# althonos/pyskani

Hardware: AMD Instinct MI355X
Metric: genome-pairs/sec (sketch+ANI) (higher is better)
Workload: dtype u64; 1 GPU; all-vs-all 10000 x 10000 synthetic ~5 Mb genomes on one GPU (100 families x 100; single-contig genomes, substitutions only), c=125 marker_c=1000 k=15; device-resident ASCII; hits=999867, genomes=10000, parallelism=references sharded over 1 GPU(s)

## Files before the change

pyskani_amd/csrc/chain.hip:

```cpp
#include "chain_stages.h"
#include "query_parts.h"
#include <hipcub/hipcub.hpp>
#include <cmath>
#include <algorithm>
#include <unordered_map>


SketchDesc make_desc(const psk_sketch* s, bool unindexed_ok) {
    SketchDesc d{};
    const bool ix = s->idx != nullptr;
    d.key = ix ? s->idx->km32 + s->idx_off : nullptr; d.pms = ix ? s->idx->pms + s->idx_off : nullptr;
    d.perm = ix ? s->idx->perm + s->idx_off : nullptr; d.bucket = ix ? s->idx->bucket + s->idx_boff : nullptr;
    d.bshift = ix ? s->idx_bshift : 0; d.n = (ix || (unindexed_ok && s->store)) ? (uint32_t)s->n_seeds : 0;
    d.pos = s->store ? s->store->seed_pos + s->seed_off : nullptr; d.meta = s->store ? s->store->seed_meta + s->seed_off : nullptr;
    d.kmer = s->store ? s->store->seed_kmer + s->seed_off : nullptr;
    d.seed_pos_base = s->store ? s->store->seed_pos : nullptr;
    d.contig_start = s->store ? s->store->contig_seed_start + s->contig_off : nullptr;
    d.total_len = s->total_len; d.n_contigs = (uint32_t)s->contig_len.size();
    uint64_t rows = 0;
    if (d.n) for (uint32_t len : s->contig_len) rows += (uint64_t)len / (FRAGMENT_LENGTH + 1) + 1;
    d.rows = (uint32_t)std::min<uint64_t>(rows, 0xFFFFFFFFu);
    s->len_quantiles(d.lenq);
    d.tab = (ix && s->ptab) ? (const ProbeLine*)s->ptab->base + s->ptab_off : nullptr; d.tab_lines = (ix && s->ptab) ? s->ptab_lines : 0;
    return d;
// ... 98 lines not shown
__global__ __launch_bounds__(256) void work_rows_kernel(const ChunkOut* __restrict__ cout, const uint32_t* __restrict__ n_chunks, const uint32_t* __restrict__ cbase,
                                                        const uint32_t* __restrict__ row_pair, uint32_t n_rows, unsigned long long* __restrict__ out) {
    __shared__ unsigned long long s_c[4], s_l[4];
    unsigned long long c = 0, live = 0;
    for (uint32_t r = blockIdx.x * blockDim.x + threadIdx.x; r < n_rows; r += gridDim.x * blockDim.x) {
        const uint32_t p = row_pair[r];
        if (r - cbase[p] < n_chunks[p]) { c += cout[r].n_cand; live++; }
    }
#pragma unroll
    for (int o = 32; o > 0; o >>= 1) { c += __shfl_xor(c, o); live += __shfl_xor(live, o); }
    if ((threadIdx.x & 63) == 0) { s_c[threadIdx.x >> 6] = c; s_l[threadIdx.x >> 6] = live; }
    __syncthreads();
    if (threadIdx.x == 0) {
        c = s_c[0] + s_c[1] + s_c[2] + s_c[3]; live = s_l[0] + s_l[1] + s_l[2] + s_l[3];
        if (live) { atomicAdd(&out[0], c); atomicAdd(&out[1], live); }
    }
}

psk_status chain_layout(Lane* ctx, size_t n_pairs, size_t n_items, size_t n_rows, size_t n_bq, ChainBufs* L) {
    const size_t gi = (n_items + 255) / 256, gi_sum = std::max(gi, (n_pairs + 3) / 4);
    size_t o_pairs = 0, o_sbase = al256(o_pairs + sizeof(PairDesc) * n_pairs), o_cbase = al256(o_sbase + 4 * (n_pairs + 1)),
           o_pstart = al256(o_cbase + 4 * (n_pairs + 1)), o_lb = al256(o_pstart + 4 * (n_pairs + 1)),
           o_aoff = al256(o_lb + 8 * (n_items + 1)), o_nch = al256(o_aoff + 4 * (n_items + 1)),
           o_chunks = al256(o_nch + 4 * n_pairs), o_rq0 = al256(o_chunks + sizeof(uint2) * n_rows), o_cout = al256(o_rq0 + sizeof(uint2) * n_rows),
           o_misc = al256(o_cout + sizeof(ChunkOut) * n_rows), o_hits = o_misc + 256, o_sel = al256(o_hits + sizeof(psk_hit) * n_pairs),
           o_ovf = al256(o_sel + sizeof(psk_hit) * n_pairs), o_bsum = al256(o_ovf + 4 * n_rows),
           o_qr = al256(o_bsum + 8 * (gi_sum + 1)), o_bq = al256(o_qr + 8 * n_pairs), o_bp = al256(o_bq + sizeof(BatchQ) * (n_bq + 1)),
           o_rp = al256(o_bp + 4 * (gi + 1)), o_live = al256(o_rp + 4 * (n_rows + 1)), o_big = al256(o_live + 4 * (n_pairs + 1)),
           o_huge = al256(o_big + 4 * (n_pairs + 1)), o_end = o_huge + 4 * (n_pairs + 1);
    PSK_TRY(ctx->q_b.reserve(o_end));
    char* B = (char*)ctx->q_b.p;
    L->pairs = (PairDesc*)(B + o_pairs); L->sbase = (uint32_t*)(B + o_sbase); L->cbase = (uint32_t*)(B + o_cbase); L->pstart = (uint32_t*)(B + o_pstart);
    L->lbcnt = (uint2*)(B + o_lb); L->aoff = (uint32_t*)(B + o_aoff); L->nch = (uint32_t*)(B + o_nch); L->chunks = (uint2*)(B + o_chunks); L->row_q0 = (uint2*)(B + o_rq0);
    L->cout = (ChunkOut*)(B + o_cout); L->hits = (psk_hit*)(B + o_hits); L->hits_sel = (psk_hit*)(B + o_sel); L->misc = (uint32_t*)(B + o_misc);
    L->ovf = (uint32_t*)(B + o_ovf); L->bsum = (unsigned long long*)(B + o_bsum); L->pair_qr = (uint2*)(B + o_qr); L->bq = (BatchQ*)(B + o_bq);
    L->blk_pair = (uint32_t*)(B + o_bp); L->row_pair = (uint32_t*)(B + o_rp); L->live = (uint32_t*)(B + o_live); L->big_list = (uint32_t*)(B + o_big); L->huge_list = (uint32_t*)(B + o_huge);
    L->gi = (uint32_t)gi; L->gi_sum = (uint32_t)gi_sum;
    L->total = (unsigned long long*)(L->misc + 16);
    return PSK_OK;
}

psk_status chain_run(Lane* ctx, const ChainBufs& L, uint32_t n_pairs, size_t n_items, size_t n_rows, const psk_params& prm,
                     const psk_query_opts* o, const SketchDesc* d_qd, const SketchDesc* d_rd, uint64_t cap, bool wide, const Switches& sw, bool probe_ok) {
    hipStream_t st = ctx->stream;
    const int force_serial = sw.chain_serial.get() != nullptr;
    const uint32_t gi = L.gi;
    hipLaunchKernelGGL(pair_table_kernel, dim3((uint32_t)(((size_t)gi + n_rows + 255) / 256)), dim3(256), 0, st, L.sbase, L.cbase, n_pairs, gi, (uint32_t)n_items, (uint32_t)n_rows, L.blk_pair, L.row_pair,
                       L.misc, L.lbcnt + n_items);
    ctx->t_begin(K_ANCHOR);
    if (wide) hipLaunchKernelGGL(anchor_count_kernel, dim3(gi), dim3(256), 0, st, L.pairs, L.sbase, n_pairs, (uint32_t)n_items, L.lbcnt, L.bsum, L.blk_pair);
    const uint32_t gi4 = (gi + JT - 1) / JT;
    uint32_t n_sum = gi;
    const int jp_force = sw.join_pairs.force();
    const bool gsi_join = !wide && (L.g_key || L.b_key) && L.d_pass && L.n_bq;
    const bool join_pairs = !wide && (gsi_join || (jp_force >= 0 ? jp_force == 1 : (n_pairs >= 16384 && n_items / n_pairs < 2048)));
    const bool gsl = gsi_join && L.gsi_slice;
    const bool gsi_one = gsi_join && !gsl && L.gsi_onepass && cap >= n_items + n_items / 8 + 8 * ((size_t)n_pairs + 1);
    bool probe_local = false;
    GsiJoinArgs GA{};
    GslArgs GL{};
    const uint32_t gsi_nw = (L.g_key && !L.gsi_slice) ? std::max(4u, (L.n_refs + 63u) / 64u) : 4u;
    const size_t gsi_lds_row = 8 * (size_t)gsi_nw + 4 * (size_t)((gsi_nw + 1u) & ~1u), gsi_lds_count = gsi_lds_row + 4 * (size_t)L.p_cap, gsi_lds_emit = gsi_lds_row + 4 * (size_t)L.p_cap * 9;
    if (gsi_join) {
        GA.bq = L.bq; GA.pass = L.d_pass; GA.n_refs = L.n_refs; GA.qd = d_qd; GA.g_key = L.g_key; GA.g_val = L.g_val; GA.g_bucket = L.g_bucket; GA.g_shift = L.g_shift;
        GA.b_key = L.b_key; GA.b_val = L.b_val; GA.b_bucket = L.b_bucket; GA.b_shift = L.b_shift; GA.b_nb1 = L.b_nb1; GA.b_blocks = L.b_blocks; GA.b_max = L.b_max;
        GA.pair_cnt = L.big_list; GA.pstart = L.pstart; GA.cap = (uint32_t)cap; GA.err = L.misc; GA.p_cap = L.p_cap; GA.nw_lds = gsi_nw;
        const uint32_t t_blocks = gsl ? L.g_blocks : L.b_blocks;
        const unsigned long long* t_base = gsl ? L.g_base : L.b_base;
        const uint32_t bcap = std::max(1u, std::min<uint32_t>(t_blocks, std::min<uint32_t>(GSI_PMAX, std::max(1u, L.p_cap))));
        uint32_t* d_btab = nullptr; uint32_t* d_bcnt = nullptr;
        if (t_blocks) {
            const size_t o_bc = al256(4 * (size_t)L.n_bq * bcap * GSL_BT_WORDS);
            PSK_TRY(ctx->q_k.reserve(o_bc + 4 * (size_t)L.n_bq + 256));
            d_btab = (uint32_t*)ctx->q_k.p; d_bcnt = (uint32_t*)((char*)ctx->q_k.p + o_bc);
            PSK_TRY(gsl_blocks_launch(L.bq, L.n_bq, L.d_pass, L.n_refs, t_blocks, t_base, d_btab, d_bcnt, bcap, st));
        }
        GA.blk_tab = d_btab; GA.blk_cnt = d_bcnt; GA.blk_cap = bcap;
        if (gsl) {
            GL.bq = L.bq; GL.n_entries = L.n_bq; GL.tab = L.gsl_tab; GL.n_tab = L.gsl_n_tab; GL.ebase = L.gsl_ebase; GL.pass = L.d_pass; GL.n_refs = L.n_refs; GL.qd = d_qd;
            GL.g_key = L.g_key; GL.g_val = L.g_val; GL.g_bucket = L.g_bucket; GL.g_shift = L.g_shift; GL.g_nb1 = L.g_nb1; GL.g_blocks = L.g_blocks; GL.g_base = L.g_base; GL.blk_tab = d_btab; GL.blk_cnt = d_bcnt; GL.blk_cap = bcap; GL.cnt = L.gsl_cnt; GL.rec = L.gsl_rec; GL.bm = L.gsl_bm; GL.un = L.gsl_un; GL.n_slices = L.gsl_n_slices;
            GL.pair_cnt = L.big_list; GL.pstart = L.pstart; GL.cap = (uint32_t)cap; GL.err = L.misc; GL.p_cap = L.p_cap; GL.chunks = L.chunks; GL.n_chunks = L.nch; GL.row_q0 = L.row_q0;
            PSK_HIP(hipMemsetAsync(L.big_list, 0, 4 * ((size_t)n_pairs + 1), st));
            PSK_TRY(gsl_count_launch(GL, st));
        }
        else if (!gsi_one) hipLaunchKernelGGL(gsi_join_kernel<false>, dim3(L.n_bq), dim3(64), gsi_lds_count, st, GA);
        probe_local = true;
    }
    else if (join_pairs) {
        size_t ts = 0;
        uint32_t* keys_in = L.big_list;
        uint32_t* vals_in = L.live;
        uint32_t* keys_out = (uint32_t*)L.hits_sel;
        uint32_t* order = keys_out + n_pairs;
        hipLaunchKernelGGL(pair_ref_keys_kernel, dim3((n_pairs + 255) / 256), dim3(256), 0, st, L.pair_qr, n_pairs, keys_in, vals_in);
        PSK_HIP(hipcub::DeviceRadixSort::SortPairs(nullptr, ts, keys_in, keys_out, vals_in, order, (int)n_pairs, 0, 32, st));
        PSK_TRY(ctx->q_g.reserve(ts + 256));
        PSK_HIP(hipcub::DeviceRadixSort::SortPairs(ctx->q_g.p, ts, keys_in, keys_out, vals_in, order, (int)n_pairs, 0, 32, st));
        const uint32_t nb = (n_pairs + 3) / 4;
        probe_local = probe_ok;
        if (probe_ok) hipLaunchKernelGGL(anchor_join_probe_kernel, dim3(nb), dim3(256), 0, st, L.pairs, L.sbase, order, n_pairs, L.lbcnt, L.bsum, L.misc + 5, L.aoff, L.big_list);
        else hipLaunchKernelGGL(anchor_join_pairs_kernel, dim3(nb), dim3(256), 0, st, L.pairs, L.sbase, order, n_pairs, L.lbcnt, L.bsum, L.misc + 5);
        n_sum = nb;
    }
    const int ep_force = sw.emit_pairs.force();
    const bool emit_pairs = !wide && !join_pairs && n_items >= 2 * ((size_t)n_pairs + 1) &&
// ... 12 lines not shown
    size_t tmp3 = 0;
    PSK_HIP(hipcub::DeviceSelect::If(nullptr, tmp3, L.hits, L.hits_sel, L.misc + 12, (int)n_pairs, HitPasses(), st));
    PSK_TRY(ctx->q_c.reserve(std::max(tmp, std::max(tmp2, tmp3))));
    unsigned long long* poff = (unsigned long long*)L.aoff;
    hipcub::TransformInputIterator<unsigned long long, Widen, const uint32_t*> pc_it(pair_cnt, Widen());
    if (gsi_one) {
        hipLaunchKernelGGL(gsi_room_kernel, dim3((n_pairs + 1 + 255) / 256), dim3(256), 0, st, (const uint32_t*)L.sbase, n_pairs, L.pstart);
        PSK_HIP(hipMemsetAsync(L.total, 0, 8, st));
    }
    else if (emit_pairs) {
        size_t tmp4 = 0;
        PSK_HIP(hipcub::DeviceScan::ExclusiveSum(nullptr, tmp4, pc_it, poff, (int)(n_pairs + 1), st));
        PSK_TRY(ctx->q_c.reserve(std::max(tmp4, std::max(tmp, std::max(tmp2, tmp3)))));
        PSK_HIP(hipcub::DeviceScan::ExclusiveSum(ctx->q_c.p, tmp4, pc_it, poff, (int)(n_pairs + 1), st));
        hipLaunchKernelGGL(pair_start64_kernel, dim3((n_pairs + 1 + 255) / 256), dim3(256), 0, st, poff, n_pairs, L.pstart, (uint32_t)cap, (const uint32_t*)(L.misc + 5));
    }
    else if (probe_local) {
        hipcub::TransformInputIterator<unsigned long long, Widen, const uint32_t*> pl_it(L.big_list, Widen());
        size_t tmp5 = 0;
        PSK_HIP(hipcub::DeviceScan::ExclusiveSum(nullptr, tmp5, pl_it, (unsigned long long*)nullptr, (int)(n_pairs + 1), st));
        const size_t o_poff = al256(tmp5 + 256);
        PSK_TRY(ctx->q_g.reserve(o_poff + 8 * ((size_t)n_pairs + 2) + 256));
        unsigned long long* pl_off64 = (unsigned long long*)((char*)ctx->q_g.p + o_poff);
        PSK_HIP(hipMemsetAsync(L.big_list + n_pairs, 0, 4, st));
        PSK_HIP(hipcub::DeviceScan::ExclusiveSum(ctx->q_g.p, tmp5, pl_it, pl_off64, (int)(n_pairs + 1), st));
        hipLaunchKernelGGL(pair_start64_kernel, dim3((n_pairs + 1 + 255) / 256), dim3(256), 0, st, (const unsigned long long*)pl_off64, n_pairs, L.pstart, (uint32_t)cap, (const uint32_t*)(L.misc + 5));
        if (gsi_join) hipLaunchKernelGGL(gsi_total_kernel, dim3(1), dim3(1), 0, st, (const unsigned long long*)pl_off64, n_pairs, L.total);
    }
    else if (wide) PSK_HIP(hipcub::DeviceScan::ExclusiveSum(ctx->q_c.p, tmp, cnt_it, L.aoff, (int)(n_items + 1), st));
    else PSK_HIP(hipcub::DeviceScan::ExclusiveSum(ctx->q_c.p, tmp, pcnt_it, L.aoff, (int)(n_items + 1), st));
    const bool small_sum = !gsi_join && n_sum <= 16384;
    if (!small_sum && !gsi_join) PSK_HIP(hipcub::DeviceReduce::Sum(ctx->q_c.p, tmp2, L.bsum, L.total, (int)n_sum, st));
    if ((!emit_pairs && !probe_local) || small_sum)
        hipLaunchKernelGGL(pair_start_kernel, dim3((emit_pairs || probe_local) ? 1u : (n_pairs + 1 + 255) / 256), dim3(256), 0, st, (emit_pairs || probe_local) ? (const uint32_t*)nullptr : L.aoff, L.sbase, n_pairs, L.pstart, (uint32_t)cap,
                           L.bsum, small_sum ? n_sum : 0u, L.total, (const uint32_t*)(L.misc + 5));
    hipLaunchKernelGGL(pair_guard_kernel, dim3((n_pairs + 1 + 255) / 256), dim3(256), 0, st, (const uint32_t*)(L.misc + 5), (const unsigned long long*)L.total, (unsigned long long)cap, L.pstart, n_pairs);
    const size_t na = ((size_t)cap + 64 + 63) & ~(size_t)63;
    PSK_TRY(ctx->q_d.reserve(4 * na * CHAIN_ANCHOR_WORDS));
    PSK_TRY(ctx->q_e.reserve(na * (8 + 4 * 7 + 1) + 512 + 4 * 2 * BIG_GMAX * (BIG_GROUPS + 64) + 4 * BIG_GROUPS));
    uint32_t* D = (uint32_t*)ctx->q_d.p;
    uint32_t* E4 = (uint32_t*)ctx->q_e.p;
    uint4* anc = (uint4*)D;
    uint32_t* a_nxt = D + 4 * na;
    ChainArgs A{};
    A.anc = anc;
    A.row_q0 = gsl ? L.row_q0 : nullptr;
    A.sc_ptr = D + 5 * na;
    A.sc_f = (int32_t*)E4; A.sc_root = E4 + na; A.sc_depth = E4 + 2 * na; A.sc_best = E4 + 3 * na;
    uint32_t* CAND = D + 6 * na;
    A.c_score.p = (int32_t*)CAND; A.c_q0.p = CAND + 1; A.c_q1.p = CAND + 2; A.c_r0.p = CAND + 3; A.c_r1.p = CAND + 4; A.c_n.p = CAND + 5; A.c_rc.p = CAND + 6; A.c_state.p = CAND + 7;
    A.chunks = L.chunks; A.n_chunks = L.nch; A.cbase = L.cbase; A.n_pairs = n_pairs; A.n_rows = (uint32_t)n_rows;
    A.row_pair = L.row_pair;
    A.pairs = L.pairs;
    A.out = L.cout; A.two_c = 2u * (uint32_t)prm.c; A.force_serial = force_serial; A.stats = L.misc + 1;
    A.band = std::max(1, std::min(MAX_CHAIN_BAND, BP_CHAIN_BAND / (int)prm.c));
    A.cap = (uint32_t)cap;
    const bool use_hops = gsi_join ? false : sw.chunk_hops.get() ? !sw.chunk_hops.off() : ((n_pairs < 1024 && n_items / n_pairs > 4096) || n_items / n_pairs > (1u << 20));
    const bool emit_heads = emit_pairs && !use_hops && !sw.emit_heads.off();
    const int hi_force = sw.hops_items.force();
    const bool hops_items = use_hops && !gsl && !emit_pairs && !join_pairs && n_items <= 0x7FFFFFFFull && (hi_force >= 0 ? hi_force == 1 : n_items / n_pairs > (1u << 20));
    ctx->t_begin(K_ANCHOR_EMIT);
    if (hops_items) {
        const size_t o_scr = al256(4 * (size_t)n_pairs * HOP_SLICES + 256);
        PSK_TRY(ctx->q_g.reserve(o_scr + sizeof(uint2) * n_rows + 256));
        uint32_t* slice_cnt = (uint32_t*)ctx->q_g.p;
        uint2* scratch_rows = (uint2*)((char*)ctx->q_g.p + o_scr);
        hipStream_t sd = nullptr;
        PSK_TRY(ctx->side_lane(&sd));
// ... 325 lines not shown
```

pyskani_amd/csrc/chain_stages.h:

```cpp
#pragma once
#include "common.h"
#include "chain_dev.h"
#include "slice_join.h"

struct PairDesc {
    const uint32_t* r_key; const uint64_t* r_pms;
    const uint32_t* q_key; const uint32_t* q_perm;
    const uint32_t* q_pos; const uint32_t* q_meta;
    const uint32_t* q_kmer;
    uint32_t q_nc, pad_;
    const uint32_t* q_seed_pos_base;
    const uint32_t* q_contig_start;
    uint64_t q_total_len, r_total_len;
    uint32_t r_n, q_n;
    const uint32_t* r_bucket; uint32_t r_bshift;
    uint32_t r_tab_lines; const ProbeLine* r_tab;
};


__device__ __forceinline__ uint32_t find_le(const uint32_t* __restrict__ base, uint32_t n, uint32_t x) {
    uint32_t lo = 0, hi = n - 1;
    while (lo < hi) { uint32_t mid = (lo + hi + 1) >> 1; if (base[mid] <= x) lo = mid; else hi = mid - 1; }
    return lo;
}
// ... 13 lines not shown

struct Widen { __host__ __device__ unsigned long long operator()(const uint32_t& v) const { return v; } };

constexpr int EP_W = 1;

constexpr int EP_T = 64 * EP_W;

constexpr int HEAD_WIN = 2048;

constexpr int HOP_WIN = 4096;

constexpr int HOP_SLICES = 32;

struct ChunkOut { uint32_t anchors, seeds, n_intervals, n_cand; uint32_t left, right; uint64_t cov_q; };

template <class T> struct Strided {
    T* p;
    __host__ __device__ __forceinline__ T& operator[](size_t i) const { return p[i * 8]; }
};

struct ChainArgs {
    const uint4* anc;
    const uint2* row_q0;
    const uint2* chunks; const uint32_t* n_chunks; const uint32_t* cbase; uint32_t n_pairs, n_rows;
    const uint32_t* row_pair;
    const uint32_t* row_order;
    const PairDesc* pairs;
    ChunkOut* out;
    int32_t* sc_f; uint32_t *sc_ptr, *sc_root, *sc_depth, *sc_best;
    Strided<int32_t> c_score; Strided<uint32_t> c_q0, c_q1, c_r0, c_r1, c_n, c_state, c_rc;
    uint32_t two_c; int band; int force_serial; int lane_dp;
    uint32_t cap;
    uint32_t* ovf_list; uint32_t* ovf_count;
    uint32_t* stats;
};

constexpr int RING = 128;

constexpr int RMAX = 256;

constexpr int CHAIN_WAVES = 4;

constexpr int LANE_N = 24;

constexpr int LANE_WAVES = 2;

// ... 72 lines not shown
constexpr int RW_PER = 8;

struct IsLivePair { const uint32_t* nch; __host__ __device__ bool operator()(const uint32_t& p) const { return nch[p] != 0; } };

struct GsiJoinArgs {
    const BatchQ* bq; const uint8_t* pass; uint32_t n_refs; const SketchDesc* qd;
    const uint32_t* g_key; const unsigned long long* g_val; const uint32_t* g_bucket; int g_shift;
    const uint32_t* b_key; const unsigned long long* b_val; const uint32_t* b_bucket; int b_shift; uint32_t b_nb1, b_blocks, b_max;
    const uint32_t* blk_tab; const uint32_t* blk_cnt; uint32_t blk_cap;
    uint32_t nw_lds;
    uint32_t* pair_cnt; const uint32_t* pstart; uint4* anc; uint32_t cap; uint32_t* err;
    uint32_t p_cap;
    uint2* chunks; uint32_t* n_chunks;
    int onepass; unsigned long long* total;
};

#ifndef LANE_NEAR_N
#define LANE_NEAR_N 3
#endif
constexpr int LANE_NEAR = LANE_NEAR_N;

__global__ __launch_bounds__(256) void pair_table_kernel(const uint32_t* __restrict__ sbase, const uint32_t* __restrict__ cbase, uint32_t n,
                                                         uint32_t n_tiles, uint32_t n_items, uint32_t n_rows,
                                                         uint32_t* __restrict__ blk_pair, uint32_t* __restrict__ row_pair, uint32_t* __restrict__ misc, uint2* __restrict__ lb_tail);
__global__ __launch_bounds__(256) void anchor_count_kernel(const PairDesc* __restrict__ pairs, const uint32_t* __restrict__ sbase,
                                                           uint32_t n_pairs, uint32_t n_items,
                                                           uint2* __restrict__ lbcnt_out, unsigned long long* __restrict__ block_sum,
                                                           const uint32_t* __restrict__ blk_pair);
__global__ __launch_bounds__(256) void anchor_join4_kernel(const PairDesc* __restrict__ pairs, const uint32_t* __restrict__ sbase,
                                                           uint32_t n_pairs, uint32_t n_items, uint32_t n_tiles,
                                                           uint2* __restrict__ item_out, unsigned long long* __restrict__ block_sum,
                                                           uint32_t* __restrict__ need_wide, const uint32_t* __restrict__ blk_pair,
                                                           uint32_t* __restrict__ pair_cnt, uint32_t xcd_group);
__global__ __launch_bounds__(256) void anchor_join_pairs_kernel(const PairDesc* __restrict__ pairs, const uint32_t* __restrict__ sbase,
                                                                const uint32_t* __restrict__ order, uint32_t n_pairs,
                                                                uint2* __restrict__ item_out, unsigned long long* __restrict__ block_sum,
                                                                uint32_t* __restrict__ need_wide);
__global__ __launch_bounds__(256) void anchor_join_probe_kernel(const PairDesc* __restrict__ pairs, const uint32_t* __restrict__ sbase,
                                                                const uint32_t* __restrict__ order, uint32_t n_pairs,
                                                                uint2* __restrict__ item_out, unsigned long long* __restrict__ block_sum,
                                                                uint32_t* __restrict__ need_wide, uint32_t* __restrict__ aoff_local, uint32_t* __restrict__ pair_cnt);
__global__ __launch_bounds__(256) void anchor_emit_packed4_kernel(const PairDesc* __restrict__ pairs, const uint32_t* __restrict__ sbase,
                                                                  uint32_t n_pairs, uint32_t n_items, uint32_t n_tiles,
                                                                  const uint2* __restrict__ item, const uint32_t* __restrict__ aoff,
                                                                  uint4* __restrict__ anc, uint32_t cap, uint32_t* __restrict__ err,
                                                                  const uint32_t* __restrict__ blk_pair, const uint32_t* __restrict__ pstart_local);
__global__ __launch_bounds__(256) void anchor_emit_expand_kernel(const PairDesc* __restrict__ pairs, const uint32_t* __restrict__ sbase,
// ... 65 lines not shown
```

pyskani_amd/csrc/join.hip:

```cpp
#include "chain_stages.h"


__global__ __launch_bounds__(256) void pair_table_kernel(const uint32_t* __restrict__ sbase, const uint32_t* __restrict__ cbase, uint32_t n,
                                                         uint32_t n_tiles, uint32_t n_items, uint32_t n_rows,
                                                         uint32_t* __restrict__ blk_pair, uint32_t* __restrict__ row_pair, uint32_t* __restrict__ misc, uint2* __restrict__ lb_tail) {
    const uint32_t t = blockIdx.x * blockDim.x + threadIdx.x;
    if (t < 64) misc[t] = 0;
    if (t == 64) *lb_tail = make_uint2(0, 0);
    if (t < n_tiles) {
        const uint64_t x = (uint64_t)t * 256u;
        blk_pair[t] = find_le(sbase, n, x < n_items ? (uint32_t)x : n_items - 1);
    } else if (t - n_tiles < n_rows) {
        row_pair[t - n_tiles] = find_le(cbase, n, t - n_tiles);
    }
}


__device__ __forceinline__ uint32_t xcd_block_id() {
    const uint32_t nb = gridDim.x, b = blockIdx.x, xcd = b & 7u, q = nb >> 3, r = nb & 7u;
    return xcd * q + (xcd < r ? xcd : r) + (b >> 3);
}

__device__ __forceinline__ uint32_t xcd_group_block_id(uint32_t g) {
    const uint32_t nb = gridDim.x, b = blockIdx.x, full = nb / (8u * g) * (8u * g);
    if (b >= full) return b;
    const uint32_t xcd = b & 7u, k = b >> 3;
    return ((k / g) * 8u + xcd) * g + (k % g);
}

__device__ __forceinline__ void lookup_lane(const uint32_t* __restrict__ key, uint32_t rn, const uint32_t* __restrict__ bucket, uint32_t bshift,
                                            uint32_t km, uint32_t& lo, uint32_t& cnt) {
// ... 1066 lines not shown
```

pyskani_amd/csrc/query_parts.h:

```cpp
#pragma once
#include "chain_stages.h"
#include <deque>
#include <vector>
#include <cstring>

static inline size_t al256(size_t x) { return (x + 255) & ~(size_t)255; }

struct SwitchVal {
    char text[24]; bool set;
    const char* get() const { return set ? text : nullptr; }
    bool off() const { return EnvVal{get()}.off(); }
    int force() const { return EnvVal{get()}.force(); }
    double num(double dflt) const { return EnvVal{get()}.num(dflt); }
};
#define PSK_SWITCHES(X) \
    X(chain_serial, "PSK_CHAIN_SERIAL") \
    X(join_pairs, "PSK_JOIN_PAIRS") \
    X(emit_pairs, "PSK_EMIT_PAIRS") \
    X(xcd_group, "PSK_XCD_GROUP") \
    X(chunk_hops, "PSK_CHUNK_HOPS") \
    X(emit_heads, "PSK_EMIT_HEADS") \
    X(hops_items, "PSK_HOPS_ITEMS") \
    X(emit_expand, "PSK_EMIT_EXPAND") \
    X(chain_lane, "PSK_CHAIN_LANE") \
// ... 28 lines not shown
    PSK_SWITCHES(X)
#undef X
    static Switches read();
    bool join_wide() const { const char* e = join.get(); return e && !strcmp(e, "wide"); }
};

struct ScreenStaging { std::deque<std::vector<MarkerSet>> hq; std::deque<std::vector<uint32_t>> qoff; };
psk_status upload_marker_table(Lane* ctx, psk_db* db);
psk_status build_inverted(Lane* ctx, psk_db* db);
psk_status screen_many_device(Lane* ctx, psk_db* db, const psk_sketch* const* queries, uint32_t nq, double screen_val, int rescue_small, uint8_t* d_pass, ScreenStaging& keep, const Switches& sw);

SketchDesc make_desc(const psk_sketch* s, bool unindexed_ok = false);
__global__ __launch_bounds__(256) void pair_build_rows_kernel(const BatchQ* __restrict__ bq, const uint8_t* __restrict__ pass, uint32_t n_refs,
                                                              const SketchDesc* __restrict__ qd, const SketchDesc* __restrict__ rd,
                                                              PairDesc* __restrict__ pairs, uint32_t* __restrict__ sbase, uint32_t* __restrict__ cbase,
                                                              uint2* __restrict__ pair_qr, uint32_t n_pairs, uint32_t n_items, uint32_t n_rows);
__global__ __launch_bounds__(256) void pass_canon_kernel(uint8_t* __restrict__ pass, uint32_t n_refs, const uint32_t* __restrict__ canon);
__global__ __launch_bounds__(256) void pass_triangle_kernel(uint8_t* __restrict__ pass, uint32_t n_refs, const long long* __restrict__ key, unsigned long long ref_base);
__global__ __launch_bounds__(256) void pass_count_kernel(const uint8_t* __restrict__ pass, uint32_t n_refs, uint32_t* __restrict__ row_count, uint8_t* __restrict__ col_flag, uint32_t* __restrict__ row_blocks);
constexpr size_t CHAIN_ANCHOR_WORDS = 14;
struct ChainBufs {
    PairDesc* pairs; uint32_t *sbase, *cbase, *pstart; uint2* lbcnt; uint32_t* aoff; uint32_t* nch; uint2* chunks; ChunkOut* cout;
    uint2* row_q0;
    psk_hit* hits; psk_hit* hits_sel; uint32_t* misc; uint32_t* ovf; unsigned long long* bsum; uint2* pair_qr; BatchQ* bq;
    uint32_t *blk_pair, *row_pair, *live, *big_list, *huge_list;
    uint32_t gi, gi_sum;
    unsigned long long* total;
    uint32_t rows_pair_max = 0xFFFFFFFFu;
    const uint32_t* g_key = nullptr; const unsigned long long* g_val = nullptr; const uint32_t* g_bucket = nullptr; int g_shift = 0;
    uint32_t g_nb1 = 0, g_blocks = 0; const unsigned long long* g_base = nullptr;
    const uint32_t* b_key = nullptr; const unsigned long long* b_val = nullptr; const uint32_t* b_bucket = nullptr; int b_shift = 0; uint32_t b_nb1 = 0, b_blocks = 0, b_max = 0; const unsigned long long* b_base = nullptr;
    const uint8_t* d_pass = nullptr; uint32_t n_refs = 0, n_bq = 0, p_cap = 0;
    bool gsi_slice = false; const uint2* gsl_tab = nullptr; uint32_t gsl_n_tab = 0; const uint2* gsl_ebase = nullptr; uint32_t *gsl_cnt = nullptr, *gsl_bm = nullptr, *gsl_un = nullptr, gsl_n_slices = 0; uint4* gsl_rec = nullptr;
    bool gsi_onepass = false;
};
psk_status chain_layout(Lane* ctx, size_t n_pairs, size_t n_items, size_t n_rows, size_t n_bq, ChainBufs* L);
psk_status chain_run(Lane* ctx, const ChainBufs& L, uint32_t n_pairs, size_t n_items, size_t n_rows, const psk_params& prm,
                     const psk_query_opts* o, const SketchDesc* d_qd, const SketchDesc* d_rd, uint64_t cap, bool wide, const Switches& sw, bool probe_ok = false);
uint64_t anchor_cap_for(Lane* ctx, size_t n_items, bool sparse = false, bool gb_scale = false);
struct ChainTail { uint32_t misc[16]; unsigned long long total64, visited, cands, rows; };
psk_status chain_check(const ChainTail& T, uint32_t n_pairs, uint64_t* cap, bool* wide, bool* retry);
static inline void count_rerun(psk_ctx* dev, bool was_wide, bool wide, bool retry) { if (wide && !was_wide) dev->rr_wide++; else if (retry) dev->rr_cap++; }
struct HostPair { const psk_sketch* r; const psk_sketch* q; };
psk_status chain_batch(Lane* ctx, const HostPair* hp, uint32_t n_pairs, const psk_query_opts* o, psk_hit* out, const Switches& sw);

uint64_t index_stamp(const psk_db* db);
// ... 9 lines not shown
```

pyskani_amd/csrc/select.hip:

```cpp
#include "chain_stages.h"



__device__ __forceinline__ void sel_commit(const SelArgs& S, uint32_t row, uint32_t q0, uint32_t q1, uint32_t n) {
    ChunkOut* o = &S.out[row];
    atomicAdd(&o->anchors, n); atomicAdd(&o->n_intervals, 1u);
    atomicMin(&o->left, q0); atomicMax(&o->right, q1);
    atomicAdd((unsigned long long*)&o->cov_q, (unsigned long long)(q1 - q0) + 1 + S.two_c);
}

__device__ void select_serial(const SelArgs& S, uint32_t row0, uint32_t nrows) {
    for (uint32_t r = 0; r < nrows; r++) { uint32_t s = S.chunks[row0 + r].x, nc = S.out[row0 + r].n_cand; for (uint32_t i = 0; i < nc; i++) S.c_state[s + i] = 0; }
    for (;;) {
        int32_t best = -1; uint32_t brow = 0, bslot = 0;
        for (uint32_t r = 0; r < nrows; r++) {
            uint32_t s = S.chunks[row0 + r].x, nc = S.out[row0 + r].n_cand;
            for (uint32_t i = 0; i < nc; i++) if (S.c_state[s + i] == 0 && S.c_score[s + i] > best) { best = S.c_score[s + i]; brow = r; bslot = s + i; }
        }
        if (best < 0) break;
        bool ok = true;
        for (uint32_t r = 0; r < nrows && ok; r++) {
            uint32_t s = S.chunks[row0 + r].x, nc = S.out[row0 + r].n_cand;
            for (uint32_t i = 0; i < nc && ok; i++) if (S.c_state[s + i] == 1) {
                uint32_t j = s + i;
// ... 539 lines not shown
    else {
        const uint32_t xcd = blockIdx.x & 7, sl = blockIdx.x >> 3, per_xcd = NB >> 3;
        if (groups >= 8) { const uint32_t gpx = groups >> 3; gid = xcd * gpx + sl / G; gr = sl % G; }
        else { gid = xcd % groups; gr = (xcd / groups) * per_xcd + sl; }
    }
    BigGrp g{G, gr, 0, B.ctr + gid, B.parts + (size_t)gid * 2 * BIG_GMAX, B.parts + (size_t)gid * 2 * BIG_GMAX + BIG_GMAX};
    for (uint32_t k = gid; k < n; k += groups) {
        select_big_pair(B, B.huge_list[k], g, s_raw, s_scan);
        __syncthreads();
    }
}

__device__ uint32_t seeds_between(const PairDesc& P, uint32_t qc, uint32_t lo, uint32_t hi) {
    const uint32_t* __restrict__ pos = P.q_seed_pos_base;
    uint32_t a = P.q_contig_start[qc], b = P.q_contig_start[qc + 1];
    uint32_t l = a, r = b;
    while (l < r) { uint32_t m = (l + r) >> 1; if (pos[m] < lo) l = m + 1; else r = m; }
    uint32_t first = l; r = b;
    if (first + 256u < b && pos[first + 256u] > hi) r = first + 256u;
    while (l < r) { uint32_t m = (l + r) >> 1; if (pos[m] <= hi) l = m + 1; else r = m; }
    return l - first;
}

__global__ __launch_bounds__(256) void chunk_seeds_kernel(ChainArgs A) {
    uint32_t row = blockIdx.x * blockDim.x + threadIdx.x;
    const uint32_t pair = A.row_pair[row < A.n_rows ? row : A.n_rows - 1];
    if (row >= A.n_rows) return;
    if (row - A.cbase[pair] >= A.n_chunks[pair]) return;
    ChunkOut* o = &A.out[row];
    if (!o->n_intervals) return;
    const uint2 ch0 = A.chunks[row];
    if (ch0.x > ch0.y || ch0.y > A.cap) return;
    const uint32_t nc = A.pairs[pair].q_nc;
    const uint32_t qc = nc == 1u ? 0u : A.row_q0 ? A.row_q0[row].y : A.anc[ch0.x].w;
    if (qc < nc) o->seeds = seeds_between(A.pairs[pair], qc, o->left, o->right);
}
```

pyskani_amd/csrc/slice_join.h:

```cpp
#pragma once
#include "common.h"

struct BatchQ { uint32_t q, rank_lo, rank_hi, pair_off, item_off, row_off; };
constexpr uint32_t GSI_PMAX = 256;

#ifndef GSL_SEEDS_N
#define GSL_SEEDS_N 256
#endif
constexpr uint32_t GSL_SEEDS = GSL_SEEDS_N;
constexpr uint32_t GSL_WORDS = GSL_SEEDS / 32;
constexpr uint32_t GSL_BT_WORDS = 12;
struct GslArgs {
    const BatchQ* bq; uint32_t n_entries;
    const uint2* tab; uint32_t n_tab;
    const uint2* ebase;
    uint32_t* un; uint32_t n_slices;
    const uint8_t* pass; uint32_t n_refs; const SketchDesc* qd;
    const uint32_t* g_key; const unsigned long long* g_val; const uint32_t* g_bucket; int g_shift;
    const unsigned long long* g_base;
    uint32_t g_nb1, g_blocks;
    uint32_t* blk_tab; uint32_t* blk_cnt; uint32_t blk_cap;
    uint32_t* cnt;
    uint4* rec;
    uint32_t* bm;
    uint32_t* pair_cnt;
    const uint32_t* pstart; uint2* anc; uint32_t cap; uint32_t* err;
    uint32_t p_cap;
    uint2* chunks; uint32_t* n_chunks;
    uint2* row_q0;
};

void gsl_make_tab(const BatchQ* bq, size_t n_entries, const uint32_t* q_seeds , std::vector<uint2>& tab, std::vector<uint2>& ebase, uint64_t* n_records, uint64_t* n_slices);
psk_status gsl_blocks_launch(const BatchQ* bq, uint32_t n_entries, const uint8_t* pass, uint32_t n_refs, uint32_t g_blocks, const unsigned long long* g_base,
                             uint32_t* blk_tab, uint32_t* blk_cnt, uint32_t blk_cap, hipStream_t st);
psk_status gsl_count_launch(const GslArgs& A, hipStream_t st);
psk_status gsl_heads_launch(const GslArgs& A, hipStream_t st);
psk_status gsl_emit_launch(const GslArgs& A, hipStream_t st);
```

pyskani_amd/csrc/slice_join.hip:

```cpp
#include "slice_join.h"
#include "chain_dev.h"

void gsl_make_tab(const BatchQ* bq, size_t n_entries, const uint32_t* q_seeds, std::vector<uint2>& tab, std::vector<uint2>& ebase, uint64_t* n_records, uint64_t* n_slices) {
    tab.clear(); ebase.resize(n_entries);
    uint64_t rec = 0, nsl_all = 0; uint32_t max_sl = 0;
    for (size_t e = 0; e < n_entries; e++) {
        const uint32_t nsl = (q_seeds[e] + GSL_SEEDS - 1) / GSL_SEEDS;
        ebase[e] = make_uint2((uint32_t)rec, (uint32_t)nsl_all);
        rec += (uint64_t)nsl * (bq[e].rank_hi - bq[e].rank_lo);
        nsl_all += nsl;
        max_sl = std::max(max_sl, nsl);
    }
    *n_records = rec; *n_slices = nsl_all;
    (void)max_sl;
    for (size_t e = 0; e < n_entries; e++) for (uint32_t sl = 0; sl < (q_seeds[e] + GSL_SEEDS - 1) / GSL_SEEDS; sl++) tab.push_back(make_uint2((uint32_t)e, sl));
}

#ifndef GSL_LINE_N
#define GSL_LINE_N 4
#endif
constexpr uint32_t GSL_LW = GSL_LINE_N, GSL_LM = GSL_LW - 1u, GSL_LS = GSL_LW == 8 ? 3u : GSL_LW == 4 ? 2u : 1u;
static_assert(GSL_LW == 8 || GSL_LW == 4 || GSL_LW == 2, "a staged line holds eight, four or two anchors");
static size_t gsl_walk_lds(const GslArgs& A, bool emit) {
    const size_t nw = (A.n_refs + 63) / 64;
    (void)nw;
    return (emit ? (8 * GSL_LW + 8 + 8) * (size_t)A.p_cap + 8 * 64 : 0) + 64 + 4 * (size_t)A.p_cap + (emit ? 0 : 4 * (size_t)GSL_WORDS * (A.p_cap + 1));
}

template <bool EMIT>
__global__ __launch_bounds__(64) void gsl_walk_kernel(GslArgs A) {
    extern __shared__ uint4 s_gsl[];
    const int lane = threadIdx.x;
    const uint2 te = A.tab[blockIdx.x];
    if (te.x == 0xFFFFFFFFu) return;
    if (EMIT && (A.err[5] || *(const unsigned long long*)(A.err + 16) > A.cap)) return;
    const BatchQ B = A.bq[te.x];
    const SketchDesc Q = A.qd[B.q];
    const uint32_t sb = te.y * GSL_SEEDS;
    if (sb >= Q.n) return;
    const uint32_t se = Q.n - sb > GSL_SEEDS ? sb + GSL_SEEDS : Q.n;
    const uint32_t P = B.rank_hi - B.rank_lo, pc = A.p_cap;
    const uint2 eb = A.ebase[te.x];
    const uint32_t rec0 = eb.x + te.y * P;
    uint2* s_line = (uint2*)s_gsl;
    unsigned long long* s_lim = (unsigned long long*)(s_line + (EMIT ? GSL_LW * pc : 0u));
    uint2* s_cs = (uint2*)(s_lim + (EMIT ? pc : 0u));
    uint2* s_fl = s_cs + (EMIT ? pc : 0u);
    uint2* s_bp = s_fl + (EMIT ? 64u : 0u);
    uint32_t* s_cur = (uint32_t*)(s_bp + 8u);
    uint32_t* s_rows = s_cur;
    uint32_t* s_bm = s_cur + pc;
    {
        if (EMIT) for (uint32_t j = lane; j < P; j += 64) { const uint4 v = A.rec[rec0 + j]; s_cs[j] = make_uint2(v.x, v.x); s_rows[j] = v.y; s_lim[j] = ((unsigned long long)v.w << 32) | v.z; }
        else {
            for (uint32_t j = lane; j < P; j += 64) s_cur[j] = 0;
            for (uint32_t x = lane; x < GSL_WORDS * (pc + 1u); x += 64) s_bm[x] = 0;
        }
    }
    uint32_t unw = 0;
    if (EMIT && lane < (int)GSL_WORDS) unw = A.un[(size_t)(eb.y + te.y) * GSL_WORDS + lane];
    lds_wave_sync();
    constexpr uint32_t GSL_AHEAD = 4;
    unsigned long long visited = 0;
    const uint32_t n_blk = A.blk_cnt[te.x];
    const uint32_t* __restrict__ brow = A.blk_tab + (size_t)te.x * A.blk_cap * GSL_BT_WORDS;
// ... 72 lines not shown
                    if (valid) { atomicAdd(&s_cur[slot], 1u); atomicOr(&s_bm[(jl >> 5) * (pc + 1u) + slot], 1u << (jl & 31u)); }
                    continue;
                }
                const uint32_t sqp = (uint32_t)__builtin_amdgcn_readlane((int)qp, (int)s), sqm = (uint32_t)__builtin_amdgcn_readlane((int)qm, (int)s);
                const uint32_t rmeta = (uint32_t)((((v >> 33) & ((1ull << GSI_CONTIG_BITS) - 1ull)) << 1) | (v & 1ull));
                const uint32_t prev = (uint32_t)__builtin_amdgcn_update_dpp(-1, (int)slot, 0x138 , 0xf, 0xf, false);
                const bool same = valid && prev == slot;
                const bool dup = __ballot(same) != 0;
                const uint2 cs = s_cs[valid ? slot : 0u];
                const unsigned long long lim = s_lim[valid ? slot : 0u];
                const uint32_t base = cs.x;
                bool opens = false;
                if (((uint32_t)__builtin_amdgcn_readlane((int)unw, (int)(jl >> 5)) >> (jl & 31u)) & 1u) {
                    const unsigned long long key1 = (((unsigned long long)(sqm >> 1) << 32) | sqp) + 1ull;
                    opens = valid && key1 > lim;
                    if (opens && !same) {
                        const uint32_t row = s_rows[slot], idxc = base < A.cap ? base : A.cap;
                        if (row < Q.rows) {
                            const size_t ri = (size_t)B.row_off + (size_t)slot * Q.rows + row;
                            uint2* r = A.chunks + ri;
                            r->x = idxc;
                            if (row > 0) r[-1].y = idxc;
                            A.row_q0[ri] = make_uint2(sqp, sqm >> 1);
                        } else atomicOr(A.err, 1u);
                        s_rows[slot] = row + 1u; s_lim[slot] = key1 + FRAGMENT_LENGTH;
                    }
                }
                const uint32_t q_rel = opens ? 0u : sqp - (uint32_t)(lim - 1ull - FRAGMENT_LENGTH);
                const uint2 av = pk_anchor(q_rel, (uint32_t)(v >> 1), (rmeta & ~1u) | ((rmeta ^ sqm) & 1u));
                if (!dup) {
                    const uint32_t t3 = base & GSL_LM;
                    if (valid) { s_cs[slot].x = base + 1u; s_line[t3 * pc + slot] = av; }
                    const bool fl = valid && t3 == GSL_LM;
                    const unsigned long long fm = __ballot(fl);
                    if (fm) {
                        if (fl) {
                            const uint32_t st0 = cs.y, lb = base & ~GSL_LM, ft = lb >= st0 ? 0u : st0 - lb;
                            s_fl[__popcll(fm & ((1ull << lane) - 1ull))] = make_uint2(slot | (ft << 16), lb);
                        }
                        lds_wave_sync();
                        const uint32_t nf = (uint32_t)__popcll(fm), t = (uint32_t)lane & GSL_LM;
                        for (uint32_t g0 = 0; g0 < nf; g0 += 64u / GSL_LW) {
                            const uint32_t r2 = g0 + ((uint32_t)lane >> GSL_LS);
                            if (r2 < nf) { const uint2 f = s_fl[r2]; if (t >= (f.x >> 16)) A.anc[f.y + t] = s_line[t * pc + (f.x & 0xFFFFu)]; }
                        }
                    }
// ... 169 lines not shown
                const unsigned long long base = g_base[blk];
                if (lane == 8) w = blk; if (lane == 9) w = run; if (lane == 10) w = (uint32_t)base; if (lane == 11) w = (uint32_t)(base >> 32);
                if (lane < (int)GSL_BT_WORDS) out[(size_t)cnt * GSL_BT_WORDS + lane] = w;
            }
            cnt++;
        }
        run += n_here;
    }
    if (lane == 0) blk_cnt[e] = cnt < blk_cap ? cnt : blk_cap;
}
psk_status gsl_blocks_launch(const BatchQ* bq, uint32_t n_entries, const uint8_t* pass, uint32_t n_refs, uint32_t g_blocks, const unsigned long long* g_base,
                             uint32_t* blk_tab, uint32_t* blk_cnt, uint32_t blk_cap, hipStream_t st) {
    if (!n_entries) return PSK_OK;
    hipLaunchKernelGGL(gsl_blocks_kernel, dim3(n_entries), dim3(64), 0, st, bq, n_entries, pass, n_refs, g_blocks, g_base, blk_tab, blk_cnt, blk_cap);
    PSK_HIP(hipGetLastError());
    return PSK_OK;
}
psk_status gsl_count_launch(const GslArgs& A, hipStream_t st) {
    hipLaunchKernelGGL(gsl_walk_kernel<false>, dim3(A.n_tab), dim3(64), gsl_walk_lds(A, false), st, A);
    PSK_HIP(hipGetLastError());
    return PSK_OK;
}
psk_status gsl_heads_launch(const GslArgs& A, hipStream_t st) {
    PSK_HIP(hipMemsetAsync(A.un, 0, 4 * (size_t)GSL_WORDS * A.n_slices, st));
    hipLaunchKernelGGL(gsl_heads_kernel, dim3(A.n_entries, (A.p_cap + 63u) / 64u), dim3(64), 0, st, A);
    PSK_HIP(hipGetLastError());
    return PSK_OK;
}
psk_status gsl_emit_launch(const GslArgs& A, hipStream_t st) {
    hipLaunchKernelGGL(gsl_walk_kernel<true>, dim3(A.n_tab), dim3(64), gsl_walk_lds(A, true), st, A);
    PSK_HIP(hipGetLastError());
    return PSK_OK;
}
```

Measured before the change: 197.1 million genome-pairs/s.

## Record chunk head seed index and bound seed search near it; fold memsets into kernels

The slice-join emit walk now records, for each chunk row, the query seed index at which the row opened. chunk_seeds_kernel uses it to binary-search only a window of up to 257 seeds after that head, instead of searching the whole contig, and falls back to the full search when the window does not cover the range. Two hipMemsetAsync calls are removed: pair_table_kernel now zeroes the pair-count list, and the count walk kernel clears its slice's bitmap words. This costs an extra per-row buffer and stores, and it relies on every slice's bitmap being visited by the count walk so that each one still gets cleared.

```diff
diff --git a/pyskani_amd/csrc/chain.hip b/pyskani_amd/csrc/chain.hip
--- a/pyskani_amd/csrc/chain.hip
+++ b/pyskani_amd/csrc/chain.hip
@@ -144,7 +144,7 @@
     size_t o_pairs = 0, o_sbase = al256(o_pairs + sizeof(PairDesc) * n_pairs), o_cbase = al256(o_sbase + 4 * (n_pairs + 1)),
            o_pstart = al256(o_cbase + 4 * (n_pairs + 1)), o_lb = al256(o_pstart + 4 * (n_pairs + 1)),
            o_aoff = al256(o_lb + 8 * (n_items + 1)), o_nch = al256(o_aoff + 4 * (n_items + 1)),
-           o_chunks = al256(o_nch + 4 * n_pairs), o_rq0 = al256(o_chunks + sizeof(uint2) * n_rows), o_cout = al256(o_rq0 + sizeof(uint2) * n_rows),
+           o_chunks = al256(o_nch + 4 * n_pairs), o_rq0 = al256(o_chunks + sizeof(uint2) * n_rows), o_rh = al256(o_rq0 + sizeof(uint2) * n_rows), o_cout = al256(o_rh + 4 * n_rows),
            o_misc = al256(o_cout + sizeof(ChunkOut) * n_rows), o_hits = o_misc + 256, o_sel = al256(o_hits + sizeof(psk_hit) * n_pairs),
            o_ovf = al256(o_sel + sizeof(psk_hit) * n_pairs), o_bsum = al256(o_ovf + 4 * n_rows),
            o_qr = al256(o_bsum + 8 * (gi_sum + 1)), o_bq = al256(o_qr + 8 * n_pairs), o_bp = al256(o_bq + sizeof(BatchQ) * (n_bq + 1)),
@@ -153,7 +153,7 @@
     PSK_TRY(ctx->q_b.reserve(o_end));
     char* B = (char*)ctx->q_b.p;
     L->pairs = (PairDesc*)(B + o_pairs); L->sbase = (uint32_t*)(B + o_sbase); L->cbase = (uint32_t*)(B + o_cbase); L->pstart = (uint32_t*)(B + o_pstart);
-    L->lbcnt = (uint2*)(B + o_lb); L->aoff = (uint32_t*)(B + o_aoff); L->nch = (uint32_t*)(B + o_nch); L->chunks = (uint2*)(B + o_chunks); L->row_q0 = (uint2*)(B + o_rq0);
+    L->lbcnt = (uint2*)(B + o_lb); L->aoff = (uint32_t*)(B + o_aoff); L->nch = (uint32_t*)(B + o_nch); L->chunks = (uint2*)(B + o_chunks); L->row_q0 = (uint2*)(B + o_rq0); L->row_h = (uint32_t*)(B + o_rh);
     L->cout = (ChunkOut*)(B + o_cout); L->hits = (psk_hit*)(B + o_hits); L->hits_sel = (psk_hit*)(B + o_sel); L->misc = (uint32_t*)(B + o_misc);
     L->ovf = (uint32_t*)(B + o_ovf); L->bsum = (unsigned long long*)(B + o_bsum); L->pair_qr = (uint2*)(B + o_qr); L->bq = (BatchQ*)(B + o_bq);
     L->blk_pair = (uint32_t*)(B + o_bp); L->row_pair = (uint32_t*)(B + o_rp); L->live = (uint32_t*)(B + o_live); L->big_list = (uint32_t*)(B + o_big); L->huge_list = (uint32_t*)(B + o_huge);
@@ -167,8 +167,9 @@
     hipStream_t st = ctx->stream;
     const int force_serial = sw.chain_serial.get() != nullptr;
     const uint32_t gi = L.gi;
-    hipLaunchKernelGGL(pair_table_kernel, dim3((uint32_t)(((size_t)gi + n_rows + 255) / 256)), dim3(256), 0, st, L.sbase, L.cbase, n_pairs, gi, (uint32_t)n_items, (uint32_t)n_rows, L.blk_pair, L.row_pair,
-                       L.misc, L.lbcnt + n_items);
+    const bool gsl_plan = !wide && (L.g_key || L.b_key) && L.d_pass && L.n_bq && L.gsi_slice;
+    hipLaunchKernelGGL(pair_table_kernel, dim3((uint32_t)((std::max((size_t)gi + n_rows, gsl_plan ? (size_t)n_pairs + 1 : (size_t)0) + 255) / 256)), dim3(256), 0, st, L.sbase, L.cbase, n_pairs, gi, (uint32_t)n_items, (uint32_t)n_rows, L.blk_pair, L.row_pair,
+                       L.misc, L.lbcnt + n_items, gsl_plan ? L.big_list : (uint32_t*)nullptr);
     ctx->t_begin(K_ANCHOR);
     if (wide) hipLaunchKernelGGL(anchor_count_kernel, dim3(gi), dim3(256), 0, st, L.pairs, L.sbase, n_pairs, (uint32_t)n_items, L.lbcnt, L.bsum, L.blk_pair);
     const uint32_t gi4 = (gi + JT - 1) / JT;
@@ -201,8 +202,7 @@
         if (gsl) {
             GL.bq = L.bq; GL.n_entries = L.n_bq; GL.tab = L.gsl_tab; GL.n_tab = L.gsl_n_tab; GL.ebase = L.gsl_ebase; GL.pass = L.d_pass; GL.n_refs = L.n_refs; GL.qd = d_qd;
             GL.g_key = L.g_key; GL.g_val = L.g_val; GL.g_bucket = L.g_bucket; GL.g_shift = L.g_shift; GL.g_nb1 = L.g_nb1; GL.g_blocks = L.g_blocks; GL.g_base = L.g_base; GL.blk_tab = d_btab; GL.blk_cnt = d_bcnt; GL.blk_cap = bcap; GL.cnt = L.gsl_cnt; GL.rec = L.gsl_rec; GL.bm = L.gsl_bm; GL.un = L.gsl_un; GL.n_slices = L.gsl_n_slices;
-            GL.pair_cnt = L.big_list; GL.pstart = L.pstart; GL.cap = (uint32_t)cap; GL.err = L.misc; GL.p_cap = L.p_cap; GL.chunks = L.chunks; GL.n_chunks = L.nch; GL.row_q0 = L.row_q0;
-            PSK_HIP(hipMemsetAsync(L.big_list, 0, 4 * ((size_t)n_pairs + 1), st));
+            GL.pair_cnt = L.big_list; GL.pstart = L.pstart; GL.cap = (uint32_t)cap; GL.err = L.misc; GL.p_cap = L.p_cap; GL.chunks = L.chunks; GL.n_chunks = L.nch; GL.row_q0 = L.row_q0; GL.row_h = L.row_h;
             PSK_TRY(gsl_count_launch(GL, st));
         }
         else if (!gsi_one) hipLaunchKernelGGL(gsi_join_kernel<false>, dim3(L.n_bq), dim3(64), gsi_lds_count, st, GA);
@@ -261,7 +261,7 @@
         const size_t o_poff = al256(tmp5 + 256);
         PSK_TRY(ctx->q_g.reserve(o_poff + 8 * ((size_t)n_pairs + 2) + 256));
         unsigned long long* pl_off64 = (unsigned long long*)((char*)ctx->q_g.p + o_poff);
-        PSK_HIP(hipMemsetAsync(L.big_list + n_pairs, 0, 4, st));
+        if (!gsl) PSK_HIP(hipMemsetAsync(L.big_list + n_pairs, 0, 4, st));
         PSK_HIP(hipcub::DeviceScan::ExclusiveSum(ctx->q_g.p, tmp5, pl_it, pl_off64, (int)(n_pairs + 1), st));
         hipLaunchKernelGGL(pair_start64_kernel, dim3((n_pairs + 1 + 255) / 256), dim3(256), 0, st, (const unsigned long long*)pl_off64, n_pairs, L.pstart, (uint32_t)cap, (const uint32_t*)(L.misc + 5));
         if (gsi_join) hipLaunchKernelGGL(gsi_total_kernel, dim3(1), dim3(1), 0, st, (const unsigned long long*)pl_off64, n_pairs, L.total);
@@ -283,6 +283,7 @@
     uint32_t* a_nxt = D + 4 * na;
     ChainArgs A{};
     A.anc = anc;
+    A.row_h = gsl ? L.row_h : nullptr;
     A.row_q0 = gsl ? L.row_q0 : nullptr;
     A.sc_ptr = D + 5 * na;
     A.sc_f = (int32_t*)E4; A.sc_root = E4 + na; A.sc_depth = E4 + 2 * na; A.sc_best = E4 + 3 * na;
diff --git a/pyskani_amd/csrc/chain_stages.h b/pyskani_amd/csrc/chain_stages.h
--- a/pyskani_amd/csrc/chain_stages.h
+++ b/pyskani_amd/csrc/chain_stages.h
@@ -59,6 +59,7 @@
 struct ChainArgs {
     const uint4* anc;
     const uint2* row_q0;
+    const uint32_t* row_h;
     const uint2* chunks; const uint32_t* n_chunks; const uint32_t* cbase; uint32_t n_pairs, n_rows;
     const uint32_t* row_pair;
     const uint32_t* row_order;
@@ -177,7 +178,8 @@
 
 __global__ __launch_bounds__(256) void pair_table_kernel(const uint32_t* __restrict__ sbase, const uint32_t* __restrict__ cbase, uint32_t n,
                                                          uint32_t n_tiles, uint32_t n_items, uint32_t n_rows,
-                                                         uint32_t* __restrict__ blk_pair, uint32_t* __restrict__ row_pair, uint32_t* __restrict__ misc, uint2* __restrict__ lb_tail);
+                                                         uint32_t* __restrict__ blk_pair, uint32_t* __restrict__ row_pair, uint32_t* __restrict__ misc, uint2* __restrict__ lb_tail,
+                                                         uint32_t* __restrict__ zero_pairs);
 __global__ __launch_bounds__(256) void anchor_count_kernel(const PairDesc* __restrict__ pairs, const uint32_t* __restrict__ sbase,
                                                            uint32_t n_pairs, uint32_t n_items,
                                                            uint2* __restrict__ lbcnt_out, unsigned long long* __restrict__ block_sum,
diff --git a/pyskani_amd/csrc/join.hip b/pyskani_amd/csrc/join.hip
--- a/pyskani_amd/csrc/join.hip
+++ b/pyskani_amd/csrc/join.hip
@@ -3,10 +3,12 @@
 
 __global__ __launch_bounds__(256) void pair_table_kernel(const uint32_t* __restrict__ sbase, const uint32_t* __restrict__ cbase, uint32_t n,
                                                          uint32_t n_tiles, uint32_t n_items, uint32_t n_rows,
-                                                         uint32_t* __restrict__ blk_pair, uint32_t* __restrict__ row_pair, uint32_t* __restrict__ misc, uint2* __restrict__ lb_tail) {
+                                                         uint32_t* __restrict__ blk_pair, uint32_t* __restrict__ row_pair, uint32_t* __restrict__ misc, uint2* __restrict__ lb_tail,
+                                                         uint32_t* __restrict__ zero_pairs) {
     const uint32_t t = blockIdx.x * blockDim.x + threadIdx.x;
     if (t < 64) misc[t] = 0;
     if (t == 64) *lb_tail = make_uint2(0, 0);
+    if (zero_pairs && t <= n) zero_pairs[t] = 0;
     if (t < n_tiles) {
         const uint64_t x = (uint64_t)t * 256u;
         blk_pair[t] = find_le(sbase, n, x < n_items ? (uint32_t)x : n_items - 1);
diff --git a/pyskani_amd/csrc/query_parts.h b/pyskani_amd/csrc/query_parts.h
--- a/pyskani_amd/csrc/query_parts.h
+++ b/pyskani_amd/csrc/query_parts.h
@@ -74,6 +74,7 @@
 struct ChainBufs {
     PairDesc* pairs; uint32_t *sbase, *cbase, *pstart; uint2* lbcnt; uint32_t* aoff; uint32_t* nch; uint2* chunks; ChunkOut* cout;
     uint2* row_q0;
+    uint32_t* row_h;
     psk_hit* hits; psk_hit* hits_sel; uint32_t* misc; uint32_t* ovf; unsigned long long* bsum; uint2* pair_qr; BatchQ* bq;
     uint32_t *blk_pair, *row_pair, *live, *big_list, *huge_list;
     uint32_t gi, gi_sum;
diff --git a/pyskani_amd/csrc/select.hip b/pyskani_amd/csrc/select.hip
--- a/pyskani_amd/csrc/select.hip
+++ b/pyskani_amd/csrc/select.hip
@@ -585,6 +585,24 @@
     return l - first;
 }
 
+__device__ uint32_t seeds_from_head(const PairDesc& P, uint32_t qc, uint32_t h, uint32_t lo, uint32_t hi) {
+    const uint32_t* __restrict__ pos = P.q_seed_pos_base;
+    const uint32_t a = P.q_contig_start[qc], b = P.q_contig_start[qc + 1];
+    const uint32_t hs = (uint32_t)(P.q_pos - pos) + h;
+    if (hs < a || hs >= b || lo > hi) return seeds_between(P, qc, lo, hi);
+    const uint32_t we = b - hs > 257u ? hs + 257u : b;
+    const uint32_t p_head = pos[hs], p_last = pos[we - 1u];
+    if (p_head > lo || p_last < lo || (p_head == lo && hs > a && pos[hs - 1u] == lo)) return seeds_between(P, qc, lo, hi);
+    uint32_t l1 = hs, r1 = we - 1u, l2 = hs, r2 = (we == b || p_last > hi) ? we : b;
+    while (l1 < r1 || l2 < r2) {
+        const uint32_t m1 = (l1 + r1) >> 1, m2 = l2 < r2 ? (l2 + r2) >> 1 : hs;
+        const uint32_t v1 = pos[m1], v2 = pos[m2];
+        if (l1 < r1) { if (v1 < lo) l1 = m1 + 1u; else r1 = m1; }
+        if (l2 < r2) { if (v2 <= hi) l2 = m2 + 1u; else r2 = m2; }
+    }
+    return l2 - l1;
+}
+
 __global__ __launch_bounds__(256) void chunk_seeds_kernel(ChainArgs A) {
     uint32_t row = blockIdx.x * blockDim.x + threadIdx.x;
     const uint32_t pair = A.row_pair[row < A.n_rows ? row : A.n_rows - 1];
@@ -596,5 +614,5 @@
     if (ch0.x > ch0.y || ch0.y > A.cap) return;
     const uint32_t nc = A.pairs[pair].q_nc;
     const uint32_t qc = nc == 1u ? 0u : A.row_q0 ? A.row_q0[row].y : A.anc[ch0.x].w;
-    if (qc < nc) o->seeds = seeds_between(A.pairs[pair], qc, o->left, o->right);
-}
+    if (qc < nc) o->seeds = A.row_h ? seeds_from_head(A.pairs[pair], qc, A.row_h[row], o->left, o->right) : seeds_between(A.pairs[pair], qc, o->left, o->right);
+}
diff --git a/pyskani_amd/csrc/slice_join.h b/pyskani_amd/csrc/slice_join.h
--- a/pyskani_amd/csrc/slice_join.h
+++ b/pyskani_amd/csrc/slice_join.h
@@ -28,6 +28,7 @@
     uint32_t p_cap;
     uint2* chunks; uint32_t* n_chunks;
     uint2* row_q0;
+    uint32_t* row_h;
 };
 
 void gsl_make_tab(const BatchQ* bq, size_t n_entries, const uint32_t* q_seeds , std::vector<uint2>& tab, std::vector<uint2>& ebase, uint64_t* n_records, uint64_t* n_slices);
diff --git a/pyskani_amd/csrc/slice_join.hip b/pyskani_amd/csrc/slice_join.hip
--- a/pyskani_amd/csrc/slice_join.hip
+++ b/pyskani_amd/csrc/slice_join.hip
@@ -41,6 +41,7 @@
     const uint32_t se = Q.n - sb > GSL_SEEDS ? sb + GSL_SEEDS : Q.n;
     const uint32_t P = B.rank_hi - B.rank_lo, pc = A.p_cap;
     const uint2 eb = A.ebase[te.x];
+    if (!EMIT && lane < (int)GSL_WORDS) A.un[(size_t)(eb.y + te.y) * GSL_WORDS + lane] = 0;
     const uint32_t rec0 = eb.x + te.y * P;
     uint2* s_line = (uint2*)s_gsl;
     unsigned long long* s_lim = (unsigned long long*)(s_line + (EMIT ? GSL_LW * pc : 0u));
@@ -159,6 +160,7 @@
                             r->x = idxc;
                             if (row > 0) r[-1].y = idxc;
                             A.row_q0[ri] = make_uint2(sqp, sqm >> 1);
+                            A.row_h[ri] = sb + jl;
                         } else atomicOr(A.err, 1u);
                         s_rows[slot] = row + 1u; s_lim[slot] = key1 + FRAGMENT_LENGTH;
                     }
@@ -374,7 +376,6 @@
     return PSK_OK;
 }
 psk_status gsl_heads_launch(const GslArgs& A, hipStream_t st) {
-    PSK_HIP(hipMemsetAsync(A.un, 0, 4 * (size_t)GSL_WORDS * A.n_slices, st));
     hipLaunchKernelGGL(gsl_heads_kernel, dim3(A.n_entries, (A.p_cap + 63u) / 64u), dim3(64), 0, st, A);
     PSK_HIP(hipGetLastError());
     return PSK_OK;
```

After: 195.8 million genome-pairs/s. About the same (-0.6%).
